# TaceoLabs/co-snarks

Measured on NVIDIA H100. Metric: co-Groth16 proofs/sec (BN254, 2^20 constraints); MSM Mscalar/s, higher is better.
Workload: dtype u32x8 (256-bit Montgomery, integer)

## Files before the change

co_snarks_b200/csrc/cs_api.cu:

```cuda
#include <stdarg.h>
#include "cs_lib.cuh"

namespace cs {

std::string& last_error() {
  static thread_local std::string e;
  return e;
}
int fail(int code, const char* fmt, ...) {
  char buf[1024];
  va_list ap;
  va_start(ap, fmt);
  vsnprintf(buf, sizeof(buf), fmt, ap);
  va_end(ap);
  last_error() = buf;
  return code;
}
#if !defined(CS_EMU)
__attribute__((constructor)) static void cs_more_hw_queues() { setenv("CUDA_DEVICE_MAX_CONNECTIONS", "32", 0); }
#endif

std::atomic<uint64_t>& launch_counter() {
  static std::atomic<uint64_t> c{0};
  return c;
// ... 155 lines not shown
int bases_upload_t(cs_ctx* ctx, const uint64_t* h_points, size_t n, int window_bits, cs_bases* b) {
  typedef typename GroupOf<Cfg, G>::F F;
  unsigned c = window_bits ? (unsigned)window_bits : msm_auto_window(n, Cfg::FR_BITS);
  if (c < 2 || c > MSM_MAX_WINDOW)
    return fail(CS_ERR_ARG, "cs_bases_upload: window_bits %d out of range [2,%u] (0 = automatic)", window_bits, MSM_MAX_WINDOW);
  b->sh = msm_shape(Cfg::FR_BITS, c);
  b->n = n;
  size_t total = (size_t)b->sh.W * n;
  if (total >= (1ull << 31)) return fail(CS_ERR_LIMIT, "cs_bases_upload: W*n = %zu exceeds 2^31", total);
  CS_TRY(b->table.reserve(total * sizeof(Affine<F>)));
  CS_CUDA(cudaMemcpyAsync(b->table.p, h_points, n * sizeof(Affine<F>), cudaMemcpyHostToDevice, ctx->stream));
  CS_TRY(b->infmask.reserve(((n + 31) / 32) * 4));
  CS_LAUNCH(k_msm_infmask<F>, ceil_div((n + 31) / 32, 128), 128, 0, ctx->stream, b->table.as<Affine<F>>(), (uint32_t)n,
            b->infmask.as<uint32_t>());
  CS_LAUNCH(k_msm_precompute<F>, ceil_div(n, 128), 128, 0, ctx->stream, b->table.as<Affine<F>>(), (uint32_t)n,
            b->sh.c, b->sh.W);
  if (G == 0 && std::is_same<Cfg, Bn254Cfg>::value) {
    static int f52_env = -1;
    if (f52_env < 0) { const char* e = getenv("CS_MSM_F52"); f52_env = e ? atoi(e) : 0; }
    if (f52_env) {
      const size_t ncoords = total * 2;
      CS_LAUNCH(k_msm_table_to_m260<Bn254Fq52 COMMA Bn254Fq>, ceil_div(ncoords, 128), 128, 0, ctx->stream,
                b->table.as<uint32_t>(), ncoords);
      b->m260 = true;
    }
  }
  CS_CUDA(cudaGetLastError());
  CS_CUDA(cudaStreamSynchronize(ctx->stream));
  return 0;
}

template <class Cfg, int G>
int msm_enqueue_t(cs_ctx* ctx, int slot, cudaStream_t st, const cs_bases* b, size_t offset,
                  const uint32_t* d_scalars, unsigned sstride, size_t n, int mont, int sort_slot, bool view) {
  typedef typename GroupOf<Cfg, G>::F F;
  return msm_enqueue<F, typename Cfg::FrP>(ctx->msm_ws[slot], b->table.as<Affine<F>>(), b->infmask.as<uint32_t>(), (uint32_t)b->n, b->sh,
                                           (uint32_t)offset, d_scalars, sstride, (uint32_t)n, mont, st,
                                           sort_slot >= 0 ? &ctx->msm_ws[sort_slot] : nullptr, view, b->m260, ctx->acc[slot]);
}

template <class Cfg, int G>
void msm_finish_t(cs_ctx* ctx, int slot, uint64_t* out_affine, int* out_inf) {
  typedef typename GroupOf<Cfg, G>::HF HF;
  const host::HXyzz<HF>* r = reinterpret_cast<const host::HXyzz<HF>*>(ctx->msm_ws[slot].h_result);
  host::HAffine<HF> a = host::haffine(*r);
  memcpy(out_affine, &a, sizeof(a));
  if (out_inf) *out_inf = a.is_inf() ? 1 : 0;
}

int msm_enqueue_dyn(cs_ctx* ctx, int slot, cudaStream_t st, const cs_bases* b, size_t offset,
                    const uint32_t* d_scalars, unsigned sstride, size_t n, int mont, int sort_slot, bool view) {
  CS_DISPATCH_CURVE(b->curve, {
    if (b->group == CS_G1) return msm_enqueue_t<Cfg, 0>(ctx, slot, st, b, offset, d_scalars, sstride, n, mont, sort_slot, view);
    return msm_enqueue_t<Cfg, 1>(ctx, slot, st, b, offset, d_scalars, sstride, n, mont, sort_slot, view);
  });
  return 0;
}
int msm_sort_shared_dyn(cs_ctx* ctx, int slot, cudaStream_t st, const cs_bases* b, const uint32_t* d_scalars,
                        unsigned sstride, size_t n, int mont) {
  CS_DISPATCH_CURVE(b->curve, {
    return msm_sort<typename Cfg::FrP>(ctx->msm_ws[slot], nullptr, (uint32_t)n, b->sh, 0, d_scalars, sstride, (uint32_t)n,
                                       mont, st);
  });
  return 0;
}

int msm_finish_dyn(cs_ctx* ctx, int slot, const cs_bases* b, uint64_t* out_affine, int* out_inf) {
  CS_DISPATCH_CURVE(b->curve, {
    if (b->group == CS_G1) msm_finish_t<Cfg, 0>(ctx, slot, out_affine, out_inf);
    else msm_finish_t<Cfg, 1>(ctx, slot, out_affine, out_inf);
  });
  return 0;
}

}

extern "C" {

int cs_bases_upload(cs_ctx* ctx, cs_curve curve, cs_group group, const uint64_t* h_points_mont, size_t n,
                    int window_bits, cs_bases** out) {
  if (!ctx || !h_points_mont || !out) return fail(CS_ERR_ARG, "cs_bases_upload: NULL argument");
  if (n == 0) return fail(CS_ERR_ARG, "cs_bases_upload: empty base set");
  if (group != CS_G1 && group != CS_G2) return fail(CS_ERR_ARG, "cs_bases_upload: bad group %d", (int)group);
  CS_CUDA(cudaSetDevice(ctx->device));
  std::unique_ptr<cs_bases> b(new cs_bases());
  b->curve = curve;
  b->group = group;
// ... 823 lines not shown
```

co_snarks_b200/csrc/cs_groth16.cu:

```cuda
#include <functional>
#include "cs_lib.cuh"
#include "cs_net.h"

using namespace cs;

struct cs_groth16_pk {
  int curve = 0;
  size_t nc = 0, ni = 0, nw = 0, n = 0;
  unsigned log_n = 0;
  DevBuf a_rowptr, a_col, a_coeff, b_rowptr, b_col, b_coeff;
  cs_bases *a_query = nullptr, *b_g1 = nullptr, *b_g2 = nullptr, *l_query = nullptr, *h_query = nullptr;
  std::vector<uint64_t> alpha_g1, beta_g1, beta_g2, delta_g1, delta_g2;
  std::vector<uint64_t> a_head, b1_head, b2_head;
  cs_domain* dom = nullptr;
  DevBuf coset_tab;
  DevBuf d_pub, d_wit, d_a, d_b, d_c, d_m1, d_m2;
  DevBuf c_rowptr, c_col, c_coeff;
  bool have_c = false;
  int wit_src[4] = {0, 1, 2, 3};
  cs_domain* dom_ark = nullptr;
  DevBuf coset_tab_ark, ginv_pows, vinv_over_n;
};

namespace {
// ... 209 lines not shown
      inf[j][i] = (words[k >> 5] >> (k & 31)) & 1;
      any = any || inf[j][i];
    }
    pk->wit_src[j] = j;
    if (q[j]->n == nw && off[j] == 0 && !any) {
      pk->wit_src[j] = -1;
      continue;
    }
    for (int k = 0; k < j; k++)
      if (pk->wit_src[k] == k && q[k]->n == q[j]->n && off[k] == off[j] && inf[k] == inf[j]) {
        pk->wit_src[j] = k;
        break;
      }
  }
  return 0;
}

int upload_inputs(cs_ctx* ctx, cs_groth16_pk* pk, int kind, const uint64_t* h_pub, const uint64_t* h_wit,
                  const uint64_t* h_m1, const uint64_t* h_m2) {
  const unsigned batch = kind == CS_REP3 ? 2 : 1;
  CS_TRY(upload(ctx, pk->d_pub, h_pub, pk->ni * 32));
  if (h_wit) CS_TRY(upload(ctx, pk->d_wit, h_wit, pk->nw * batch * 32));
  if (kind == CS_REP3 && h_m1) CS_TRY(upload(ctx, pk->d_m1, h_m1, pk->n * 32));
  if (kind == CS_REP3 && h_m2) CS_TRY(upload(ctx, pk->d_m2, h_m2, pk->n * 32));
  return 0;
}

template <class Cfg>
int local_phase(cs_ctx* ctx, cs_groth16_pk* pk, int kind, int party, const uint64_t* h_pub, const uint64_t* h_wit,
                const uint64_t* d_wit_in, const uint64_t* h_m1, const uint64_t* h_m2, const uint64_t* r_hs, const uint64_t* s_hs,
                uint64_t* out_a, uint64_t* out_b1, uint64_t* out_b2, uint64_t* out_l, uint64_t* out_h,
                unsigned parts = CS_PART_ALL, const cs_rep3_prf* prf = nullptr, const uint64_t* rs_mont = nullptr,
                uint64_t* out_rs_delta = nullptr, const std::function<void()>* overlap = nullptr,
                const std::function<int(const uint64_t*, const uint64_t*)>* mid = nullptr) {
  typedef HostGroup<Cfg, 0> H1;
  typedef HostGroup<Cfg, 1> H2;
  const unsigned batch = kind == CS_REP3 ? 2 : 1;
  const bool add_public = (kind == CS_PLAIN) || party == 0;
  const bool have_aux = pk->nw > 0;
  const bool do_a = parts & CS_PART_A, do_b1 = parts & CS_PART_B1, do_b2 = parts & CS_PART_B2,
             do_l = parts & CS_PART_L, do_h = parts & CS_PART_H;
  CS_CUDA(cudaSetDevice(ctx->device));
  CS_TRY(upload_inputs(ctx, pk, kind, h_pub, h_wit, do_h ? h_m1 : nullptr, do_h ? h_m2 : nullptr));
  CS_TRY(ctx_fork(ctx, 5));
  cudaStream_t wm = ctx->wm;
  CS_CUDA(cudaStreamWaitEvent(wm, ctx->ev_fork, 0));
  const uint32_t* wit = d_wit_in ? reinterpret_cast<const uint32_t*>(d_wit_in) : pk->d_wit.as<uint32_t>();
  if (do_h) {
    bool have_m1 = h_m1 != nullptr, have_m2 = h_m2 != nullptr;
    if (prf && kind == CS_REP3) {
      typedef typename Cfg::FrP FrP;
      const size_t n = pk->n;
      CS_TRY(pk->d_m1.reserve(n * 32));
      CS_TRY(pk->d_m2.reserve(n * 32));
      CS_TRY(ctx->prf_keys.reserve(64));
      CS_CUDA(cudaMemcpyAsync(ctx->prf_keys.p, prf->seed1, 32, cudaMemcpyHostToDevice, wm));
      CS_CUDA(cudaMemcpyAsync((char*)ctx->prf_keys.p + 32, prf->seed2, 32, cudaMemcpyHostToDevice, wm));
      CS_LAUNCH(k_rep3_masks<FrP>, ceil_div(n, 128), 128, 0, wm, ctx->prf_keys.as<uint32_t>(), prf->word_pos1,
                prf->word_pos2, prf->rounds, n, pk->d_m1.as<uint32_t>());
      CS_LAUNCH(k_rep3_masks<FrP>, ceil_div(n, 128), 128, 0, wm, ctx->prf_keys.as<uint32_t>(),
                prf->word_pos1 + 8 * n, prf->word_pos2 + 8 * n, prf->rounds, n, pk->d_m2.as<uint32_t>());
      have_m1 = have_m2 = true;
    }
    CS_TRY((witness_map_device<Cfg>(ctx, pk, kind, party, wit, have_m1, have_m2, wm)));
    {
      CS_SPAN("msm h_query");
      CS_TRY(msm_enqueue_dyn(ctx, 4, wm, pk->h_query, 0, pk->d_c.as<uint32_t>(), 1, pk->n, 1));
    }
  }
  if (have_aux) {
    CS_SPAN("compute A, B/G1, B/G2 in create proof with assignment + msm l_query");
    const unsigned part[4] = {CS_PART_A, CS_PART_B1, CS_PART_B2, CS_PART_L};
    const cs_bases* q[4] = {pk->a_query, pk->b_g1, pk->b_g2, pk->l_query};
    const size_t off[4] = {pk->ni, pk->ni, pk->ni, 0};
    if (do_a || do_b1 || do_b2 || do_l)
      CS_TRY(msm_sort_shared_dyn(ctx, CS_WIT_SORT, ctx->side[4], pk->a_query, wit, batch, pk->nw, 1));
    for (int j = 0; j < 4; j++) {
      if (!(parts & part[j])) continue;
      int src = pk->wit_src[j];
      if (src >= 0 && !(parts & part[src])) src = j;
      const int sort_slot = src < 0 || src == j ? CS_WIT_SORT : src;
      CS_TRY(msm_enqueue_dyn(ctx, j, ctx->side[j], q[j], off[j], wit, batch, pk->nw, 1, sort_slot, src == j));
    }
  }
  CS_TRY(ctx_join(ctx, 5));
  CS_CUDA(cudaEventRecord(ctx->ev_wm, wm));
  CS_CUDA(cudaStreamWaitEvent(ctx->stream, ctx->ev_wm, 0));

  const size_t g1l = 2 * H1::HF::N, g2l = 4 * H1::HF::N;
  typename H1::X a_acc = H1::X::inf(), b1_acc = H1::X::inf();
  typename H2::X b2_acc = H2::X::inf();
  if (do_a) {
    a_acc = H1::mul(H1::load(pk->delta_g1.data()), r_hs);
    if (add_public) {
      a_acc = host::hadd(a_acc, H1::load(pk->a_head.data()));
      a_acc = host::hadd(a_acc, H1::load(pk->alpha_g1.data()));
      for (size_t k = 1; k < pk->ni; k++)
        a_acc = host::hadd(a_acc, H1::mul(H1::load(pk->a_head.data() + k * g1l), h_pub + k * 4));
    }
  }
  if (do_b1) {
    b1_acc = H1::mul(H1::load(pk->delta_g1.data()), s_hs);
    if (add_public) {
      b1_acc = host::hadd(b1_acc, H1::load(pk->b1_head.data()));
      b1_acc = host::hadd(b1_acc, H1::load(pk->beta_g1.data()));
      for (size_t k = 1; k < pk->ni; k++)
        b1_acc = host::hadd(b1_acc, H1::mul(H1::load(pk->b1_head.data() + k * g1l), h_pub + k * 4));
    }
  }
  if (do_b2) {
    b2_acc = H2::mul(H2::load(pk->delta_g2.data()), s_hs);
    if (add_public) {
      b2_acc = host::hadd(b2_acc, H2::load(pk->b2_head.data()));
      b2_acc = host::hadd(b2_acc, H2::load(pk->beta_g2.data()));
      for (size_t k = 1; k < pk->ni; k++)
        b2_acc = host::hadd(b2_acc, H2::mul(H2::load(pk->b2_head.data() + k * g2l), h_pub + k * 4));
    }
  }
  CS_SPAN("r*s without networking");
  if (rs_mont && out_rs_delta)
    H1::store(out_rs_delta, H1::mul(H1::load(pk->delta_g1.data()), rs_mont));
  if (overlap) (*overlap)();
  uint64_t tmp[24];
  int inf = 0;
  bool ab_done = false;
  if (mid && have_aux && do_a && do_b1) {
    CS_CUDA(cudaEventSynchronize(ctx->ev_side[0]));
    CS_CUDA(cudaEventSynchronize(ctx->ev_side[1]));
    CS_TRY(msm_finish_dyn(ctx, 0, pk->a_query, tmp, &inf)); a_acc = host::hadd(a_acc, H1::load(tmp));
    CS_TRY(msm_finish_dyn(ctx, 1, pk->b_g1, tmp, &inf)); b1_acc = host::hadd(b1_acc, H1::load(tmp));
    H1::store(out_a, a_acc);
    H1::store(out_b1, b1_acc);
    CS_TRY((*mid)(out_a, out_b1));
    ab_done = true;
  }
  CS_CUDA(cudaStreamSynchronize(ctx->stream));
  memset(out_l, 0, g1l * 8);
  memset(out_h, 0, g1l * 8);
  if (have_aux) {
    if (do_a && !ab_done) { CS_TRY(msm_finish_dyn(ctx, 0, pk->a_query, tmp, &inf)); a_acc = host::hadd(a_acc, H1::load(tmp)); }
    if (do_b1 && !ab_done) { CS_TRY(msm_finish_dyn(ctx, 1, pk->b_g1, tmp, &inf)); b1_acc = host::hadd(b1_acc, H1::load(tmp)); }
    if (do_b2) { CS_TRY(msm_finish_dyn(ctx, 2, pk->b_g2, tmp, &inf)); b2_acc = host::hadd(b2_acc, H2::load(tmp)); }
    if (do_l) CS_TRY(msm_finish_dyn(ctx, 3, pk->l_query, out_l, &inf));
  }
  if (do_h) CS_TRY(msm_finish_dyn(ctx, 4, pk->h_query, out_h, &inf));
  if (!ab_done) {
    H1::store(out_a, a_acc);
    H1::store(out_b1, b1_acc);
  }
  H2::store(out_b2, b2_acc);
  if (mid && !ab_done) CS_TRY((*mid)(out_a, out_b1));
  return 0;
}

template <class Cfg>
int prove_plain_t(cs_ctx* ctx, cs_groth16_pk* pk, const uint64_t* h_pub, const uint64_t* h_wit,
                  const uint64_t* d_wit, const uint64_t* r, const uint64_t* s, uint64_t* out_a, uint64_t* out_b,
                  uint64_t* out_c) {
  typedef HostGroup<Cfg, 0> H1;
  typedef host::HFp<typename Cfg::FrP> HR;
  uint64_t a[12], b1[12], l[12], h[12], rsd[12];
  HR rr, ss;
  memcpy(rr.l, r, sizeof(rr.l));
  memcpy(ss.l, s, sizeof(ss.l));
  HR rs = rr * ss;
  typename H1::X c = H1::X::inf();
  std::function<int(const uint64_t*, const uint64_t*)> mid = [&](const uint64_t* pa, const uint64_t* pb1) -> int {
    c = host::hadd(H1::mul(H1::load(pa), s), H1::mul(H1::load(pb1), r));
    return 0;
  };
  CS_TRY((local_phase<Cfg>(ctx, pk, CS_PLAIN, 0, h_pub, h_wit, d_wit, nullptr, nullptr, r, s, a, b1, out_b, l, h,
                           CS_PART_ALL, nullptr, rs.l, rsd, nullptr, &mid)));
  c = host::hadd(c, host::hneg(H1::load(rsd)));
  c = host::hadd(c, H1::load(l));
  c = host::hadd(c, H1::load(h));
  memcpy(out_a, a, 2 * H1::HF::N * 8);
  H1::store(out_c, c);
  return 0;
}


template <class Cfg>
int rep3_prove_t(cs_ctx* ctx, cs_groth16_pk* pk, cs_net* net0, cs_net* net1, cs_net* pair, int role, int party,
                 cs_rep3_state* state0, const uint64_t* h_pub, const uint64_t* h_wit, const uint64_t* d_wit,
                 uint64_t* out_a, uint64_t* out_b, uint64_t* out_c, uint64_t* out_rs) {
  typedef HostGroup<Cfg, 0> H1;
  typedef HostGroup<Cfg, 1> H2;
  typedef host::HFp<typename Cfg::FrP> HR;
  typedef typename Cfg::FrP FrP;
  constexpr size_t G1L = 2 * H1::HF::N, G2L = 4 * H1::HF::N;
  const size_t n = pk->n;
  cs_rep3_state* st1p = nullptr;
  CS_TRY(cs_rep3_state_fork(state0, &st1p));
  std::unique_ptr<cs_rep3_state> state1(st1p);
  cs_rep3_prf prf;
  CS_TRY(cs_rep3_state_prf(state0, &prf));
  CS_TRY(cs_rep3_state_advance(state0, 16 * (uint64_t)n));
  uint64_t r_sh[2 * HR::N], s_sh[2 * HR::N];
  CS_TRY(cs_rep3_state_rand(state0, (cs_curve)pk->curve, r_sh));
  CS_TRY(cs_rep3_state_rand(state0, (cs_curve)pk->curve, s_sh));
  if (out_rs) { memcpy(out_rs, r_sh, sizeof(r_sh)); memcpy(out_rs + 2 * HR::N, s_sh, sizeof(s_sh)); }
  HR ra, rb, sa, sb;
  memcpy(ra.l, r_sh, sizeof(ra.l)); memcpy(rb.l, r_sh + HR::N, sizeof(rb.l));
  memcpy(sa.l, s_sh, sizeof(sa.l)); memcpy(sb.l, s_sh + HR::N, sizeof(sb.l));
  HR m1 = state0->rng1.template fr_be_mod_order<FrP>(), m2 = state0->rng2.template fr_be_mod_order<FrP>();
// ... 10 lines not shown
    memcpy(msg + G2L, h, G1L * 8);
    return cs_net_send(pair, 0, msg, sizeof(msg));
  }
  typename H1::X ec_mask = H1::X::inf();
  std::function<void()> overlap = [&]() {
    typename H1::X g = H1::load(pk->alpha_g1.data());
    HR a1, a2;
    memcpy(a1.l, k1, sizeof(a1.l)); memcpy(a2.l, k2, sizeof(a2.l));
    HR d = a1 - a2;
    HR dc = d.from_mont();
    ec_mask = host::hmul(g, dc.l, HR::N);
  };
  uint64_t g_a[G1L], g1_b[G1L], g2_b[G2L], l_acc[G1L], h_acc[G1L], rsd[G1L];
  const unsigned parts = role == 1 ? (CS_PART_A | CS_PART_B1 | CS_PART_L) : CS_PART_ALL;
  Rep3Net n0(net0), n1(net1);
  typename H1::X A_open = H1::X::inf(), g_c = H1::X::inf();
  std::function<int(const uint64_t*, const uint64_t*)> mid = [&](const uint64_t* pa, const uint64_t* pb1) -> int {
    CS_SPAN("network round after calc coeff");
    CS_TRY(n0.send_next(pa, G1L * 8));
    CS_TRY(n0.send_prev(pa, G1L * 8));
    CS_TRY(n1.send_next(pb1, G1L * 8));
    typename H1::X B1 = H1::load(pb1);
    typename H1::X t = H1::mul(B1, r_sh + HR::N);
    uint64_t ga_prev[G1L], ga_next[G1L], g1b_prev[G1L];
    CS_TRY(n0.recv_prev(ga_prev, G1L * 8));
    CS_TRY(n0.recv_next(ga_next, G1L * 8));
    CS_TRY(n1.recv_prev(g1b_prev, G1L * 8));
    A_open = host::hadd(host::hadd(H1::load(pa), H1::load(ga_prev)), H1::load(ga_next));
    typename H1::X r_g1_b = host::hadd(host::hadd(H1::mul(host::hadd(B1, H1::load(g1b_prev)), r_sh), t), ec_mask);
    g_c = host::hadd(H1::mul(A_open, s_sh), r_g1_b);
    return 0;
  };
  CS_TRY((local_phase<Cfg>(ctx, pk, CS_REP3, party, h_pub, h_wit, d_wit, nullptr, nullptr, r_sh, s_sh, g_a, g1_b, g2_b,
                           l_acc, h_acc, parts, role == 1 ? nullptr : &prf, rs.l, rsd, &overlap, &mid)));
  if (role == 1) {
    uint64_t msg[G2L + G1L];
    CS_TRY(cs_net_recv(pair, 1, msg, sizeof(msg)));
    memcpy(g2_b, msg, G2L * 8);
    memcpy(h_acc, msg + G2L, G1L * 8);
  }
  CS_SPAN("finish - open two points and some adds");
  g_c = host::hadd(g_c, host::hneg(H1::load(rsd)));
  g_c = host::hadd(g_c, H1::load(l_acc));
  g_c = host::hadd(g_c, H1::load(h_acc));
  uint64_t gc[G1L];
  H1::store(gc, g_c);
  CS_TRY(n0.send_next(gc, G1L * 8));
  CS_TRY(n0.send_prev(gc, G1L * 8));
  CS_TRY(n1.send_next(g2_b, G2L * 8));
  CS_TRY(n1.send_prev(g2_b, G2L * 8));
  uint64_t gc_prev[G1L], gc_next[G1L], b2_prev[G2L], b2_next[G2L];
  CS_TRY(n0.recv_prev(gc_prev, G1L * 8));
  CS_TRY(n0.recv_next(gc_next, G1L * 8));
  CS_TRY(n1.recv_prev(b2_prev, G2L * 8));
  CS_TRY(n1.recv_next(b2_next, G2L * 8));
  H1::store(out_a, A_open);
  H1::store(out_c, host::hadd(host::hadd(g_c, H1::load(gc_prev)), H1::load(gc_next)));
  H2::store(out_b, host::hadd(host::hadd(H2::load(g2_b), H2::load(b2_prev)), H2::load(b2_next)));
  return 0;
}

template <class Cfg>
int shamir_prove_t(cs_ctx* ctx, cs_groth16_pk* pk, cs_net* net0, cs_net* net1, int n_parties, int threshold,
                   const uint64_t* h_pub, const uint64_t* h_wit, const uint64_t* d_wit, uint64_t* out_a, uint64_t* out_b,
                   uint64_t* out_c, uint64_t* out_rs) {
  typedef HostGroup<Cfg, 0> H1;
  typedef host::HFp<typename Cfg::FrP> HR;
  constexpr size_t G1L = 2 * H1::HF::N, G2L = 4 * H1::HF::N;
  cs_shamir_state* s0 = nullptr;
  CS_TRY(cs_shamir_state_create(net0, (cs_curve)pk->curve, n_parties, threshold, 3, &s0));
  struct Guard { cs_shamir_state* a = nullptr; cs_shamir_state* b = nullptr; ~Guard() { cs_shamir_state_free(a); cs_shamir_state_free(b); } } guard;
  guard.a = s0;
  cs_shamir_state* s1 = nullptr;
  CS_TRY(cs_shamir_state_fork(s0, 1, &s1));
  guard.b = s1;
  uint64_t r[HR::N], sv[HR::N];
  CS_TRY(cs_shamir_state_rand(s0, net0, r));
  CS_TRY(cs_shamir_state_rand(s0, net0, sv));
  if (out_rs) { memcpy(out_rs, r, sizeof(r)); memcpy(out_rs + HR::N, sv, sizeof(sv)); }
  HR rr, ss;
  memcpy(rr.l, r, sizeof(r));
  memcpy(ss.l, sv, sizeof(sv));
  HR rs = rr * ss;
  uint64_t g_a[G1L], g1_b[G1L], g2_b[G2L], l_acc[G1L], h_acc[G1L], rsd[G1L];
  CS_TRY((local_phase<Cfg>(ctx, pk, CS_PLAIN, 0, h_pub, h_wit, d_wit, nullptr, nullptr, r, sv, g_a, g1_b, g2_b, l_acc, h_acc,
                           CS_PART_ALL, nullptr, rs.l, rsd)));
  uint64_t a_open[G1L], g1_b_red[G1L];
  CS_TRY(cs_shamir_open_half_point(s0, net0, CS_G1, g_a, a_open));
  CS_TRY(cs_shamir_degree_reduce_point(s1, net1, CS_G1, pk->alpha_g1.data(), g1_b, g1_b_red));
  typename H1::X r_g1_b = H1::mul(H1::load(g1_b_red), r);
  typename H1::X g_c = H1::mul(H1::load(a_open), sv);
  g_c = host::hadd(g_c, r_g1_b);
  g_c = host::hadd(g_c, host::hneg(H1::load(rsd)));
  g_c = host::hadd(g_c, H1::load(l_acc));
  g_c = host::hadd(g_c, H1::load(h_acc));
  uint64_t gc[G1L];
  H1::store(gc, g_c);
  CS_TRY(cs_shamir_open_half_point(s0, net0, CS_G1, gc, out_c));
  CS_TRY(cs_shamir_open_half_point(s1, net1, CS_G2, g2_b, out_b));
  memcpy(out_a, a_open, sizeof(a_open));
  return 0;
}

int rep3_prove_dispatch(cs_ctx* ctx, cs_groth16_pk* pk, cs_net* net0, cs_net* net1, cs_net* pair, int role, int party,
                        cs_rep3_state* state, const uint64_t* h_pub, const uint64_t* h_wit, const uint64_t* d_wit,
                        uint64_t* out_a, uint64_t* out_b, uint64_t* out_c, uint64_t* out_rs) {
  if (!ctx || !pk || !state || !h_pub) return fail(CS_ERR_ARG, "cs_groth16_rep3_prove: NULL argument");
  if (pk->nw && !h_wit == !d_wit) return fail(CS_ERR_ARG, "cs_groth16_rep3_prove: pass the witness shares either on the host or on the device");
  if (role != 2) {
    if (!net0 || !net1 || !out_a || !out_b || !out_c) return fail(CS_ERR_ARG, "cs_groth16_rep3_prove: NULL argument");
    if (net0->n != 3 || net1->n != 3 || net0->id != net1->id) return fail(CS_ERR_ARG, "cs_groth16_rep3_prove: net0/net1 must be 3-party meshes of the same party");
    if (net0->id != state->id) return fail(CS_ERR_ARG, "cs_groth16_rep3_prove: state belongs to party %d, net to party %d", state->id, net0->id);
  }
  if (role != 0 && (!pair || pair->n != 2 || pair->id != role - 1)) return fail(CS_ERR_ARG, "cs_groth16_rep3_prove: pair must be the 2-party link (id %d)", role - 1);
  if (party < 0 || party > 2) return fail(CS_ERR_ARG, "cs_groth16_rep3_prove: party must be 0..2");
  switch (pk->curve) {
    case CS_BN254:
      return rep3_prove_t<Bn254Cfg>(ctx, pk, net0, net1, pair, role, party, state, h_pub, h_wit, d_wit, out_a, out_b, out_c, out_rs);
#if defined(CS_ENABLE_BLS12_381)
// ... 314 lines not shown
```

co_snarks_b200/csrc/cs_lib.cuh:

```cuda
#pragma once
#include <atomic>
#include <map>
#include <memory>
#include "cs_common.cuh"
#include "cs_params.cuh"
#include "cs_curve.cuh"
#include "cs_msm.cuh"
#include "cs_msm52.cuh"
#include "cs_ntt.cuh"
#include "cs_ntt8.cuh"
#include "cs_vec.cuh"
#include "cs_prf.cuh"
#include "cs_host_field.h"
#include "../../include/cosnarks_gpu.h"

namespace cs {

struct Bn254Cfg {
  typedef Bn254Fq FqP;
  typedef Bn254Fr FrP;
  static constexpr unsigned FR_BITS = 254;
  static constexpr unsigned TWO_ADICITY = 28;
};
struct Bls381Cfg {
// ... 52 lines not shown
  unsigned log_n = 0;
  cs::DevBuf tw_fwd, tw_inv;
  cs::DevBuf inv_n;
  std::vector<uint64_t> group_gen;
};

#if defined(CS_ENABLE_BLS12_381)
#define CS_CASE_BLS(...)   \
  case CS_BLS12_381: {     \
    typedef Bls381Cfg Cfg; \
    __VA_ARGS__;           \
  } break;
#else
#define CS_CASE_BLS(...)
#endif

#define CS_DISPATCH_CURVE(curve, ...)                                        \
  switch ((int)(curve)) {                                                    \
    case CS_BN254: {                                                         \
      typedef Bn254Cfg Cfg;                                                  \
      __VA_ARGS__;                                                           \
    } break;                                                                 \
      CS_CASE_BLS(__VA_ARGS__)                                               \
    default:                                                                 \
      return cs::fail(CS_ERR_ARG, "unsupported curve id %d", (int)(curve));      \
  }


namespace cs {
std::atomic<uint64_t>& launch_counter();
int ctx_fork(cs_ctx* ctx, int nside);
int ctx_join(cs_ctx* ctx, int nside);
int msm_enqueue_dyn(cs_ctx* ctx, int slot, cudaStream_t st, const cs_bases* b, size_t offset,
                    const uint32_t* d_scalars, unsigned sstride, size_t n, int mont, int sort_slot = -1, bool view = false);
int msm_sort_shared_dyn(cs_ctx* ctx, int slot, cudaStream_t st, const cs_bases* b, const uint32_t* d_scalars,
                        unsigned sstride, size_t n, int mont);
int msm_finish_dyn(cs_ctx* ctx, int slot, const cs_bases* b, uint64_t* out_affine, int* out_inf);
int ntt_run(cs_ctx* ctx, const cs_domain* d, uint32_t* d_data, unsigned batch, bool inverse_in_to_out,
            const uint32_t* d_post, cudaStream_t st);
}
```

co_snarks_b200/csrc/cs_msm.cuh:

```cuda
#pragma once
#include <stdlib.h>
#include "cs_common.cuh"
#include "cs_curve.cuh"

namespace cs {

constexpr unsigned MSM_SLICE_MAX = 64;
constexpr unsigned MSM_ORDER_BLOCK = 256;
constexpr unsigned MSM_RED_SEG = 4;
constexpr unsigned MSM_SIGN = 0x80000000u;

template <class FrP>
CS_GLOBAL void k_msm_digits(const uint32_t* __restrict__ scalars, uint32_t sstride, uint32_t n, int mont,
                            uint32_t c, uint32_t W, const uint32_t* __restrict__ infmask, uint32_t offset,
                            uint32_t* __restrict__ dig, uint32_t* __restrict__ count) {
  uint32_t i = blockIdx.x * blockDim.x + threadIdx.x;
  if (i >= n) return;
  if (infmask && ((infmask[(offset + i) >> 5] >> ((offset + i) & 31)) & 1)) {
    for (uint32_t w = 0; w < W; w++) dig[(size_t)w * n + i] = 0;
    return;
  }
  Fp<FrP> s;
  const uint4* src = reinterpret_cast<const uint4*>(scalars) + (size_t)i * sstride * (FrP::N / 4);
  CS_UNROLL
// ... 351 lines not shown
  }
  Affine<F> p = table[e & ~MSM_SIGN];
  for (uint32_t k = beg; k < end; k++) {
    uint32_t e_cur = e;
    Affine<F> p_cur = p;
    if (k + 1 < end) {
      e = sorted[k + 1];
      p = table[e & ~MSM_SIGN];
    }
    madd(acc, p_cur, (e_cur & MSM_SIGN) != 0);
  }
  part0[s] = acc;
}

template <class F>
CS_GLOBAL void __launch_bounds__(128) k_msm_accum1(const Xyzz<F>* __restrict__ part0,
                                                   const uint32_t* __restrict__ sstart0,
                                                   const uint32_t* __restrict__ sstart1, uint32_t nb1, uint32_t S,
                                                   Xyzz<F>* __restrict__ part1) {
  uint32_t s = blockIdx.x * blockDim.x + threadIdx.x;
  if (s >= sstart1[nb1]) return;
  uint32_t b = find_bucket(sstart1, nb1, s);
  uint32_t j = s - sstart1[b];
  uint32_t beg = sstart0[b] + j * S;
  uint32_t end = sstart0[b + 1];
  if (end > beg + S) end = beg + S;
  Xyzz<F> acc = part0[beg];
  for (uint32_t k = beg + 1; k < end; k++) padd(acc, part0[k]);
  part1[s] = acc;
}

template <class F>
CS_GLOBAL void __launch_bounds__(128) k_msm_accum2(const Xyzz<F>* __restrict__ part1,
                                                   const uint32_t* __restrict__ sstart1, uint32_t nb1,
                                                   Xyzz<F>* __restrict__ bucket) {
  uint32_t b = blockIdx.x * blockDim.x + threadIdx.x;
  if (b >= nb1) return;
  uint32_t beg = sstart1[b], end = sstart1[b + 1];
  Xyzz<F> acc = Xyzz<F>::inf();
  if (beg < end) {
    acc = part1[beg];
    for (uint32_t k = beg + 1; k < end; k++) padd(acc, part1[k]);
  }
  bucket[b] = acc;
}

template <class F>
CS_GLOBAL void __launch_bounds__(128) k_msm_reduce_seg(const Xyzz<F>* __restrict__ bucket, uint32_t B,
                                                       uint32_t L, Xyzz<F>* __restrict__ red) {
  uint32_t t = blockIdx.x * blockDim.x + threadIdx.x;
  uint32_t lo = t * L;
  if (lo >= B) return;
  uint32_t hi = lo + L < B ? lo + L : B;
  Xyzz<F> acc = Xyzz<F>::inf(), tot = Xyzz<F>::inf();
  for (uint32_t b = hi; b > lo; b--) {
    padd(acc, bucket[b]);
    padd(tot, acc);
  }
  if (lo != 0 && !acc.is_inf()) {
    Xyzz<F> m = Xyzz<F>::inf();
    int top = 31 - __clz(lo);
    for (int bit = top; bit >= 0; bit--) {
      m = dbl_xyzz(m);
      if ((lo >> bit) & 1) padd(m, acc);
    }
    padd(tot, m);
  }
  red[t] = tot;
}

template <class F>
CS_GLOBAL void k_msm_final_sum(const Xyzz<F>* __restrict__ red, uint32_t cnt,
                                                      Xyzz<F>* __restrict__ out) {
  CS_DYN_SMEM(Xyzz<F>, sm);
  const uint32_t T = blockDim.x, t = threadIdx.x;
  Xyzz<F> acc = Xyzz<F>::inf();
// ... 81 lines not shown
  Xyzz<F> acc = Xyzz<F>::inf();
  for (int bit = FrP::N * 32 - 1; bit >= 0; bit--) {
    acc = dbl_xyzz(acc);
    if ((lim[bit >> 5] >> (bit & 31)) & 1) madd(acc, b, false);
  }
  out[i] = to_affine(acc);
}

struct MsmShape {
  uint32_t c, W, B;
};

static inline MsmShape msm_shape(uint32_t scalar_bits, uint32_t c) {
  MsmShape s;
  s.c = c;
  s.W = (scalar_bits + 1 + c - 1) / c;
  s.B = 1u << (c - 1);
  return s;
}

static inline uint32_t msm_auto_window(size_t n, uint32_t scalar_bits) {
  int lg = 0;
  while ((1ull << (lg + 1)) <= n) lg++;
  int c = lg >= 15 ? 16 : lg - 4;
  if (c < 4) c = 4;
  while (c < 16) {
    const uint32_t W = (scalar_bits + 1 + c - 1) / c;
    const uint32_t top = scalar_bits + 1 - (W - 1) * c;
    if (2 * top >= (uint32_t)c) break;
    c++;
  }
  return (uint32_t)c;
}
static inline uint32_t msm_slice(const MsmShape& sh) {
  const char* e = getenv("CS_MSM_SLICE");
  if (e && atoi(e) == 64) return 64u;
  if (e && atoi(e) == 32) return 32u;
  return sh.c >= 18 ? 64u : 32u;
}

constexpr int MSM_NSTAGE = 5;
struct MsmWorkspace {
  DevBuf dig, sorted, meta, part0, part1, part2, bucket, red, scal, result, order;
  void* h_result = nullptr;
  size_t h_result_cap = 0;
  bool profile = false;
  cudaEvent_t ev[MSM_NSTAGE + 1] = {};
  cudaEvent_t sorted_ev = nullptr;
  bool sorted_ev_made = false, sorted_once = false;
  cudaEvent_t acc_in = nullptr, acc_out = nullptr;
  int mark(int i, cudaStream_t st) {
    if (!profile) return 0;
    if (!ev[i]) CS_CUDA(cudaEventCreateWithFlags(&ev[i], 0));
    CS_CUDA(cudaEventRecord(ev[i], st));
    return 0;
  }
  void release() {
    for (int i = 0; i <= MSM_NSTAGE; i++) {
      if (ev[i]) cudaEventDestroy(ev[i]);
      ev[i] = nullptr;
    }
    if (sorted_ev_made) cudaEventDestroy(sorted_ev);
    if (acc_in) cudaEventDestroy(acc_in);
    if (acc_out) cudaEventDestroy(acc_out);
    acc_in = acc_out = nullptr;
    sorted_ev = nullptr;
    sorted_ev_made = sorted_once = false;
    dig.release(); sorted.release(); meta.release(); part0.release(); part1.release(); part2.release();
    bucket.release(); red.release(); scal.release(); result.release(); order.release();
    if (h_result) cudaFreeHost(h_result);
    h_result = nullptr;
    h_result_cap = 0;
  }
};

template <class F>
int msm_accum0_f52(const Affine<F>* table, const uint32_t* sorted, const uint32_t* count, const uint32_t* start,
                   const uint32_t* sstart0, uint32_t nb1, uint32_t S, const uint32_t* order, const uint32_t* order_b,
                   Xyzz<F>* part0, uint32_t max_s0, cudaStream_t st);

struct MsmSizes {
  uint32_t nb1, S, ob;
  size_t nent, max_s0, max_s1, max_s2;
  MsmSizes(const MsmShape& sh, uint32_t n) {
    nb1 = sh.B + 1;
    nent = (size_t)sh.W * n;
    S = msm_slice(sh);
    max_s0 = nent / S + nb1;
    max_s1 = max_s0 / S + nb1;
    max_s2 = max_s1 / S + nb1;
    ob = ceil_div(max_s0, MSM_ORDER_BLOCK);
  }
  size_t meta_words() const { return 2 * (size_t)nb1 + 4 * ((size_t)nb1 + 1) + 4 * MSM_SCAN_MAX_BLOCKS; }
  size_t order_words() const {
    return 4 * max_s0 + (size_t)ob * (MSM_SLICE_MAX + 1) + 2 * (MSM_SLICE_MAX + 1) + (size_t)(MSM_SLICE_MAX + 1) * MSM_OFF_CHUNKS;
  }
};
struct MsmSortBufs {
  uint32_t *count, *cursor, *start, *sstart0, *sstart1, *sstart2, *aux;
  uint32_t *slice_len, *slice_bkt, *order, *order_b, *block_hist, *len_base, *chunk_sum;
  MsmSortBufs(const MsmWorkspace& w, const MsmSizes& z) {
    count = w.meta.as<uint32_t>();
    cursor = count + z.nb1;
    start = cursor + z.nb1;
    sstart0 = start + z.nb1 + 1;
    sstart1 = sstart0 + z.nb1 + 1;
    sstart2 = sstart1 + z.nb1 + 1;
    aux = sstart2 + z.nb1 + 1;
    slice_len = w.order.as<uint32_t>();
    slice_bkt = slice_len + z.max_s0;
    order = slice_bkt + z.max_s0;
    order_b = order + z.max_s0;
    block_hist = order_b + z.max_s0;
    len_base = block_hist + (size_t)z.ob * (MSM_SLICE_MAX + 1);
    chunk_sum = len_base + 2 * (MSM_SLICE_MAX + 1);
  }
};

static inline int msm_check_limits(const MsmShape& sh, uint32_t n, uint32_t nbases) {
  const size_t nent = (size_t)sh.W * n;
// ... 45 lines not shown
  CS_TRY(ws.mark(1, st));
  CS_TRY(msm_scan(q, z, sh.B, st));
  CS_LAUNCH(k_msm_scatter, dim3(ceil_div(n, 256), sh.W), 256, 0, st, ws.dig.as<uint32_t>(), n, nbases, offset, q.start,
            q.cursor, ws.sorted.as<uint32_t>());
  return msm_slice_order(ws, q, z, st);
}

static inline int msm_view(MsmWorkspace& ws, const MsmWorkspace& src, const uint32_t* infmask, uint32_t nbases,
                           MsmShape sh, uint32_t offset, uint32_t n, cudaStream_t st) {
  const MsmSizes z(sh, n);
  const uint32_t nblk = ceil_div(z.nent, MSM_VIEW_T);
  CS_TRY(ws.dig.reserve(((size_t)nblk * MSM_VIEW_WORDS + 2 * (size_t)nblk + 1) * 4));
  CS_TRY(ws.sorted.reserve(z.nent * 4));
  CS_TRY(ws.meta.reserve(z.meta_words() * 4));
  CS_TRY(ws.order.reserve(z.order_words() * 4));
  const MsmSortBufs q(ws, z), s(src, z);
  uint32_t* keep = ws.dig.as<uint32_t>();
  uint32_t* blk_cnt = keep + (size_t)nblk * MSM_VIEW_WORDS;
  uint32_t* blk_off = blk_cnt + nblk;
  const uint32_t* src_sorted = src.sorted.as<uint32_t>();
  CS_LAUNCH_SYNC(k_msm_view_flags, nblk, MSM_VIEW_T, 0, st, src_sorted, s.start, z.nb1, n, infmask, offset, keep, blk_cnt);
  CS_LAUNCH_SYNC(k_msm_view_scan, 1, MSM_SCAN_T, 0, st, blk_cnt, nblk, blk_off);
  CS_LAUNCH(k_msm_view_counts, ceil_div(z.nb1, 256), 256, 0, st, s.start, z.nb1, keep, blk_off, q.count);
  CS_LAUNCH(k_msm_view_scatter, nblk, MSM_VIEW_T, 0, st, src_sorted, n, nbases, offset, keep, blk_off,
            ws.sorted.as<uint32_t>());
  CS_TRY(msm_scan(q, z, sh.B, st));
  return msm_slice_order(ws, q, z, st);
}

template <class F, class FrP>
int msm_enqueue(MsmWorkspace& ws, const Affine<F>* table, const uint32_t* infmask, uint32_t nbases, MsmShape sh,
                uint32_t offset,
                const uint32_t* d_scalars, uint32_t sstride, uint32_t n, int mont, cudaStream_t st,
                MsmWorkspace* sort_from = nullptr, bool view = false, bool table_m260 = false, cudaStream_t st_acc = nullptr) {
  CS_TRY(msm_check_limits(sh, n, nbases));
  const MsmSizes z(sh, n);
  const uint32_t nb1 = z.nb1, S = z.S;
  const size_t max_s0 = z.max_s0, max_s1 = z.max_s1, max_s2 = z.max_s2;
  CS_TRY(ws.part0.reserve(max_s0 * sizeof(Xyzz<F>)));
  CS_TRY(ws.part1.reserve(max_s1 * sizeof(Xyzz<F>)));
  CS_TRY(ws.part2.reserve(max_s2 * sizeof(Xyzz<F>)));
  CS_TRY(ws.bucket.reserve((size_t)nb1 * sizeof(Xyzz<F>)));
  const uint32_t L = sh.B < MSM_RED_SEG ? sh.B : MSM_RED_SEG;
  const uint32_t nseg = (sh.B + L - 1) / L;
  const uint32_t fs_threads = sizeof(Xyzz<F>) > 128 ? 128 : 256;
  const uint32_t fs_blocks = nseg > 4 * fs_threads ? (nseg + fs_threads - 1) / fs_threads : 1;
  CS_TRY(ws.red.reserve(((size_t)nseg + fs_blocks) * sizeof(Xyzz<F>)));
  CS_TRY(ws.result.reserve(sizeof(Xyzz<F>)));
  if (ws.h_result_cap < sizeof(Xyzz<F>)) {
    if (ws.h_result) cudaFreeHost(ws.h_result);
    CS_CUDA(cudaMallocHost(&ws.h_result, sizeof(Xyzz<F>)));
    ws.h_result_cap = sizeof(Xyzz<F>);
  }
  if (sort_from) {
    if (!sort_from->sorted_once) return fail(-1, "msm: the workspace to share a sort with has not been enqueued");
    CS_TRY(ws.mark(0, st));
    CS_CUDA(cudaStreamWaitEvent(st, sort_from->sorted_ev, 0));
    CS_TRY(ws.mark(1, st));
    if (view) CS_TRY(msm_view(ws, *sort_from, infmask, nbases, sh, offset, n, st));
  } else {
    CS_TRY(msm_sort<FrP>(ws, infmask, nbases, sh, offset, d_scalars, sstride, n, mont, st));
  }
  MsmWorkspace& so = sort_from && !view ? *sort_from : ws;
  const MsmSortBufs q(so, z);
  const uint32_t *count = q.count, *start = q.start, *sstart0 = q.sstart0, *sstart1 = q.sstart1, *sstart2 = q.sstart2;
  const uint32_t *order = q.order, *order_b = q.order_b;
  CS_TRY(ws.mark(2, st));
// ... 8 lines not shown
    st = st_acc;
  }
  {
    static int minb_env = -1;
    if (minb_env < 0) { const char* e = getenv("CS_ACCUM0_MINB"); minb_env = e ? atoi(e) : 0; }
    const int minb = minb_env ? minb_env : (sizeof(Affine<F>) > 64 ? 2 : 4);
    if (table_m260) {
      CS_TRY((msm_accum0_f52<F>(table, so.sorted.as<uint32_t>(), count, start, sstart0, nb1, S, order, order_b,
                                ws.part0.as<Xyzz<F>>(), (uint32_t)max_s0, st)));
    } else {
#define CS_ACC0(M)                                                                                              \
  CS_LAUNCH(k_msm_accum0<F COMMA M>, ceil_div(max_s0, 128), 128, 0, st, table, so.sorted.as<uint32_t>(), count, \
            start, sstart0, nb1, S, order, order_b, ws.part0.as<Xyzz<F>>())
    switch (minb) {
      case 2: CS_ACC0(2); break;
      case 3: CS_ACC0(3); break;
      case 5: CS_ACC0(5); break;
      case 6: CS_ACC0(6); break;
      default: CS_ACC0(4); break;
    }
#undef CS_ACC0
    }
  }
  if (st_acc) {
    CS_CUDA(cudaEventRecord(ws.acc_out, st_acc));
    st = st_main;
    CS_CUDA(cudaStreamWaitEvent(st, ws.acc_out, 0));
  }
  CS_TRY(ws.mark(3, st));
  CS_LAUNCH(k_msm_accum1<F>, ceil_div(max_s1, 128), 128, 0, st, ws.part0.as<Xyzz<F>>(), sstart0, sstart1,
            nb1, S, ws.part1.as<Xyzz<F>>());
  CS_LAUNCH(k_msm_accum1<F>, ceil_div(max_s2, 128), 128, 0, st, ws.part1.as<Xyzz<F>>(), sstart1, sstart2,
            nb1, S, ws.part2.as<Xyzz<F>>());
  CS_LAUNCH(k_msm_accum2<F>, ceil_div(nb1, 128), 128, 0, st, ws.part2.as<Xyzz<F>>(), sstart2, nb1,
            ws.bucket.as<Xyzz<F>>());
  CS_TRY(ws.mark(4, st));
  CS_LAUNCH(k_msm_reduce_seg<F>, ceil_div(nseg, 128), 128, 0, st, ws.bucket.as<Xyzz<F>>(), sh.B, L,
            ws.red.as<Xyzz<F>>());
  if (fs_blocks > 1) {
    Xyzz<F>* stage = ws.red.as<Xyzz<F>>() + nseg;
    CS_LAUNCH_SYNC(k_msm_final_sum<F>, fs_blocks, fs_threads, fs_threads * sizeof(Xyzz<F>), st, ws.red.as<Xyzz<F>>(), nseg,
                   stage);
    CS_LAUNCH_SYNC(k_msm_final_sum<F>, 1, fs_threads, fs_threads * sizeof(Xyzz<F>), st, stage, fs_blocks,
                   ws.result.as<Xyzz<F>>());
  } else {
    CS_LAUNCH_SYNC(k_msm_final_sum<F>, 1, fs_threads, fs_threads * sizeof(Xyzz<F>), st, ws.red.as<Xyzz<F>>(), nseg,
                   ws.result.as<Xyzz<F>>());
  }
  CS_TRY(ws.mark(5, st));
  CS_CUDA(cudaMemcpyAsync(ws.h_result, ws.result.p, sizeof(Xyzz<F>), cudaMemcpyDeviceToHost, st));
  CS_CUDA(cudaGetLastError());
  return 0;
}

}
```

Measured before the change: 49.69.

## Fold H-query MSM partial buckets into L-query MSM to share reduction tail

Result: faster. 50.73, median of 6 (+2.1%).

```diff
diff --git a/co_snarks_b200/csrc/cs_api.cu b/co_snarks_b200/csrc/cs_api.cu
--- a/co_snarks_b200/csrc/cs_api.cu
+++ b/co_snarks_b200/csrc/cs_api.cu
@@ -211,11 +211,13 @@
 
 template <class Cfg, int G>
 int msm_enqueue_t(cs_ctx* ctx, int slot, cudaStream_t st, const cs_bases* b, size_t offset,
-                  const uint32_t* d_scalars, unsigned sstride, size_t n, int mont, int sort_slot, bool view) {
+                  const uint32_t* d_scalars, unsigned sstride, size_t n, int mont, int sort_slot, bool view,
+                  bool defer_tail, int fold_slot) {
   typedef typename GroupOf<Cfg, G>::F F;
   return msm_enqueue<F, typename Cfg::FrP>(ctx->msm_ws[slot], b->table.as<Affine<F>>(), b->infmask.as<uint32_t>(), (uint32_t)b->n, b->sh,
                                            (uint32_t)offset, d_scalars, sstride, (uint32_t)n, mont, st,
-                                           sort_slot >= 0 ? &ctx->msm_ws[sort_slot] : nullptr, view, b->m260, ctx->acc[slot]);
+                                           sort_slot >= 0 ? &ctx->msm_ws[sort_slot] : nullptr, view, b->m260, ctx->acc[slot],
+                                           defer_tail, fold_slot >= 0 ? &ctx->msm_ws[fold_slot] : nullptr);
 }
 
 template <class Cfg, int G>
@@ -228,10 +230,12 @@
 }
 
 int msm_enqueue_dyn(cs_ctx* ctx, int slot, cudaStream_t st, const cs_bases* b, size_t offset,
-                    const uint32_t* d_scalars, unsigned sstride, size_t n, int mont, int sort_slot, bool view) {
+                    const uint32_t* d_scalars, unsigned sstride, size_t n, int mont, int sort_slot, bool view,
+                    bool defer_tail, int fold_slot) {
   CS_DISPATCH_CURVE(b->curve, {
-    if (b->group == CS_G1) return msm_enqueue_t<Cfg, 0>(ctx, slot, st, b, offset, d_scalars, sstride, n, mont, sort_slot, view);
-    return msm_enqueue_t<Cfg, 1>(ctx, slot, st, b, offset, d_scalars, sstride, n, mont, sort_slot, view);
+    if (b->group == CS_G1)
+      return msm_enqueue_t<Cfg, 0>(ctx, slot, st, b, offset, d_scalars, sstride, n, mont, sort_slot, view, defer_tail, fold_slot);
+    return msm_enqueue_t<Cfg, 1>(ctx, slot, st, b, offset, d_scalars, sstride, n, mont, sort_slot, view, defer_tail, fold_slot);
   });
   return 0;
 }
diff --git a/co_snarks_b200/csrc/cs_groth16.cu b/co_snarks_b200/csrc/cs_groth16.cu
--- a/co_snarks_b200/csrc/cs_groth16.cu
+++ b/co_snarks_b200/csrc/cs_groth16.cu
@@ -265,7 +265,7 @@
                 uint64_t* out_a, uint64_t* out_b1, uint64_t* out_b2, uint64_t* out_l, uint64_t* out_h,
                 unsigned parts = CS_PART_ALL, const cs_rep3_prf* prf = nullptr, const uint64_t* rs_mont = nullptr,
                 uint64_t* out_rs_delta = nullptr, const std::function<void()>* overlap = nullptr,
-                const std::function<int(const uint64_t*, const uint64_t*)>* mid = nullptr) {
+                const std::function<int(const uint64_t*, const uint64_t*)>* mid = nullptr, bool sum_lh = false) {
   typedef HostGroup<Cfg, 0> H1;
   typedef HostGroup<Cfg, 1> H2;
   const unsigned batch = kind == CS_REP3 ? 2 : 1;
@@ -273,6 +273,8 @@
   const bool have_aux = pk->nw > 0;
   const bool do_a = parts & CS_PART_A, do_b1 = parts & CS_PART_B1, do_b2 = parts & CS_PART_B2,
              do_l = parts & CS_PART_L, do_h = parts & CS_PART_H;
+  const bool merge_lh = sum_lh && have_aux && do_l && do_h && pk->l_query->sh.c == pk->h_query->sh.c &&
+                        pk->l_query->sh.W == pk->h_query->sh.W;
   CS_CUDA(cudaSetDevice(ctx->device));
   CS_TRY(upload_inputs(ctx, pk, kind, h_pub, h_wit, do_h ? h_m1 : nullptr, do_h ? h_m2 : nullptr));
   CS_TRY(ctx_fork(ctx, 5));
@@ -298,7 +300,7 @@
     CS_TRY((witness_map_device<Cfg>(ctx, pk, kind, party, wit, have_m1, have_m2, wm)));
     {
       CS_SPAN("msm h_query");
-      CS_TRY(msm_enqueue_dyn(ctx, 4, wm, pk->h_query, 0, pk->d_c.as<uint32_t>(), 1, pk->n, 1));
+      CS_TRY(msm_enqueue_dyn(ctx, 4, wm, pk->h_query, 0, pk->d_c.as<uint32_t>(), 1, pk->n, 1, -1, false, merge_lh));
     }
   }
   if (have_aux) {
@@ -313,7 +315,8 @@
       int src = pk->wit_src[j];
       if (src >= 0 && !(parts & part[src])) src = j;
       const int sort_slot = src < 0 || src == j ? CS_WIT_SORT : src;
-      CS_TRY(msm_enqueue_dyn(ctx, j, ctx->side[j], q[j], off[j], wit, batch, pk->nw, 1, sort_slot, src == j));
+      CS_TRY(msm_enqueue_dyn(ctx, j, ctx->side[j], q[j], off[j], wit, batch, pk->nw, 1, sort_slot, src == j, false,
+                             j == 3 && merge_lh ? 4 : -1));
     }
   }
   CS_TRY(ctx_join(ctx, 5));
@@ -376,7 +379,7 @@
     if (do_b2) { CS_TRY(msm_finish_dyn(ctx, 2, pk->b_g2, tmp, &inf)); b2_acc = host::hadd(b2_acc, H2::load(tmp)); }
     if (do_l) CS_TRY(msm_finish_dyn(ctx, 3, pk->l_query, out_l, &inf));
   }
-  if (do_h) CS_TRY(msm_finish_dyn(ctx, 4, pk->h_query, out_h, &inf));
+  if (do_h && !merge_lh) CS_TRY(msm_finish_dyn(ctx, 4, pk->h_query, out_h, &inf));
   if (!ab_done) {
     H1::store(out_a, a_acc);
     H1::store(out_b1, b1_acc);
@@ -403,7 +406,7 @@
     return 0;
   };
   CS_TRY((local_phase<Cfg>(ctx, pk, CS_PLAIN, 0, h_pub, h_wit, d_wit, nullptr, nullptr, r, s, a, b1, out_b, l, h,
-                           CS_PART_ALL, nullptr, rs.l, rsd, nullptr, &mid)));
+                           CS_PART_ALL, nullptr, rs.l, rsd, nullptr, &mid, true)));
   c = host::hadd(c, host::hneg(H1::load(rsd)));
   c = host::hadd(c, H1::load(l));
   c = host::hadd(c, H1::load(h));
@@ -480,7 +483,7 @@
     return 0;
   };
   CS_TRY((local_phase<Cfg>(ctx, pk, CS_REP3, party, h_pub, h_wit, d_wit, nullptr, nullptr, r_sh, s_sh, g_a, g1_b, g2_b,
-                           l_acc, h_acc, parts, role == 1 ? nullptr : &prf, rs.l, rsd, &overlap, &mid)));
+                           l_acc, h_acc, parts, role == 1 ? nullptr : &prf, rs.l, rsd, &overlap, &mid, true)));
   if (role == 1) {
     uint64_t msg[G2L + G1L];
     CS_TRY(cs_net_recv(pair, 1, msg, sizeof(msg)));
@@ -532,7 +535,7 @@
   HR rs = rr * ss;
   uint64_t g_a[G1L], g1_b[G1L], g2_b[G2L], l_acc[G1L], h_acc[G1L], rsd[G1L];
   CS_TRY((local_phase<Cfg>(ctx, pk, CS_PLAIN, 0, h_pub, h_wit, d_wit, nullptr, nullptr, r, sv, g_a, g1_b, g2_b, l_acc, h_acc,
-                           CS_PART_ALL, nullptr, rs.l, rsd)));
+                           CS_PART_ALL, nullptr, rs.l, rsd, nullptr, nullptr, true)));
   uint64_t a_open[G1L], g1_b_red[G1L];
   CS_TRY(cs_shamir_open_half_point(s0, net0, CS_G1, g_a, a_open));
   CS_TRY(cs_shamir_degree_reduce_point(s1, net1, CS_G1, pk->alpha_g1.data(), g1_b, g1_b_red));
diff --git a/co_snarks_b200/csrc/cs_lib.cuh b/co_snarks_b200/csrc/cs_lib.cuh
--- a/co_snarks_b200/csrc/cs_lib.cuh
+++ b/co_snarks_b200/csrc/cs_lib.cuh
@@ -108,7 +108,8 @@
 int ctx_fork(cs_ctx* ctx, int nside);
 int ctx_join(cs_ctx* ctx, int nside);
 int msm_enqueue_dyn(cs_ctx* ctx, int slot, cudaStream_t st, const cs_bases* b, size_t offset,
-                    const uint32_t* d_scalars, unsigned sstride, size_t n, int mont, int sort_slot = -1, bool view = false);
+                    const uint32_t* d_scalars, unsigned sstride, size_t n, int mont, int sort_slot = -1, bool view = false,
+                    bool defer_tail = false, int fold_slot = -1);
 int msm_sort_shared_dyn(cs_ctx* ctx, int slot, cudaStream_t st, const cs_bases* b, const uint32_t* d_scalars,
                         unsigned sstride, size_t n, int mont);
 int msm_finish_dyn(cs_ctx* ctx, int slot, const cs_bases* b, uint64_t* out_affine, int* out_inf);
diff --git a/co_snarks_b200/csrc/cs_msm.cuh b/co_snarks_b200/csrc/cs_msm.cuh
--- a/co_snarks_b200/csrc/cs_msm.cuh
+++ b/co_snarks_b200/csrc/cs_msm.cuh
@@ -407,7 +407,9 @@
 
 template <class F>
 CS_GLOBAL void __launch_bounds__(128) k_msm_accum2(const Xyzz<F>* __restrict__ part1,
-                                                   const uint32_t* __restrict__ sstart1, uint32_t nb1,
+                                                   const uint32_t* __restrict__ sstart1,
+                                                   const Xyzz<F>* __restrict__ part_b,
+                                                   const uint32_t* __restrict__ sstart_b, uint32_t nb1,
                                                    Xyzz<F>* __restrict__ bucket) {
   uint32_t b = blockIdx.x * blockDim.x + threadIdx.x;
   if (b >= nb1) return;
@@ -417,6 +419,8 @@
     acc = part1[beg];
     for (uint32_t k = beg + 1; k < end; k++) padd(acc, part1[k]);
   }
+  if (part_b)
+    for (uint32_t k = sstart_b[b]; k < sstart_b[b + 1]; k++) padd(acc, part_b[k]);
   bucket[b] = acc;
 }
 
@@ -564,11 +568,11 @@
   }
   return (uint32_t)c;
 }
-static inline uint32_t msm_slice(const MsmShape& sh) {
+static inline uint32_t msm_slice(const MsmShape& sh, size_t nent) {
   const char* e = getenv("CS_MSM_SLICE");
   if (e && atoi(e) == 64) return 64u;
   if (e && atoi(e) == 32) return 32u;
-  return sh.c >= 18 ? 64u : 32u;
+  return sh.c >= 18 || (sh.c >= 16 && nent >= 255 * (size_t)sh.B) ? 64u : 32u;
 }
 
 constexpr int MSM_NSTAGE = 5;
@@ -581,6 +585,10 @@
   cudaEvent_t sorted_ev = nullptr;
   bool sorted_ev_made = false, sorted_once = false;
   cudaEvent_t acc_in = nullptr, acc_out = nullptr;
+  cudaEvent_t part_ev = nullptr;
+  bool part_ev_made = false;
+  const uint32_t* part_sstart2 = nullptr;
+  uint32_t part_nb1 = 0;
   int mark(int i, cudaStream_t st) {
     if (!profile) return 0;
     if (!ev[i]) CS_CUDA(cudaEventCreateWithFlags(&ev[i], 0));
@@ -595,7 +603,11 @@
     if (sorted_ev_made) cudaEventDestroy(sorted_ev);
     if (acc_in) cudaEventDestroy(acc_in);
     if (acc_out) cudaEventDestroy(acc_out);
-    acc_in = acc_out = nullptr;
+    if (part_ev_made) cudaEventDestroy(part_ev);
+    acc_in = acc_out = part_ev = nullptr;
+    part_ev_made = false;
+    part_sstart2 = nullptr;
+    part_nb1 = 0;
     sorted_ev = nullptr;
     sorted_ev_made = sorted_once = false;
     dig.release(); sorted.release(); meta.release(); part0.release(); part1.release(); part2.release();
@@ -617,7 +629,7 @@
   MsmSizes(const MsmShape& sh, uint32_t n) {
     nb1 = sh.B + 1;
     nent = (size_t)sh.W * n;
-    S = msm_slice(sh);
+    S = msm_slice(sh, nent);
     max_s0 = nent / S + nb1;
     max_s1 = max_s0 / S + nb1;
     max_s2 = max_s1 / S + nb1;
@@ -729,7 +741,8 @@
 int msm_enqueue(MsmWorkspace& ws, const Affine<F>* table, const uint32_t* infmask, uint32_t nbases, MsmShape sh,
                 uint32_t offset,
                 const uint32_t* d_scalars, uint32_t sstride, uint32_t n, int mont, cudaStream_t st,
-                MsmWorkspace* sort_from = nullptr, bool view = false, bool table_m260 = false, cudaStream_t st_acc = nullptr) {
+                MsmWorkspace* sort_from = nullptr, bool view = false, bool table_m260 = false, cudaStream_t st_acc = nullptr,
+                bool defer_tail = false, MsmWorkspace* fold_in = nullptr) {
   CS_TRY(msm_check_limits(sh, n, nbases));
   const MsmSizes z(sh, n);
   const uint32_t nb1 = z.nb1, S = z.S;
@@ -804,7 +817,29 @@
             nb1, S, ws.part1.as<Xyzz<F>>());
   CS_LAUNCH(k_msm_accum1<F>, ceil_div(max_s2, 128), 128, 0, st, ws.part1.as<Xyzz<F>>(), sstart1, sstart2,
             nb1, S, ws.part2.as<Xyzz<F>>());
-  CS_LAUNCH(k_msm_accum2<F>, ceil_div(nb1, 128), 128, 0, st, ws.part2.as<Xyzz<F>>(), sstart2, nb1,
+  if (defer_tail) {
+    if (!ws.part_ev_made) {
+      CS_CUDA(cudaEventCreateWithFlags(&ws.part_ev, cudaEventDisableTiming));
+      ws.part_ev_made = true;
+    }
+    CS_CUDA(cudaEventRecord(ws.part_ev, st));
+    ws.part_sstart2 = sstart2;
+    ws.part_nb1 = nb1;
+    CS_TRY(ws.mark(4, st));
+    CS_TRY(ws.mark(5, st));
+    CS_CUDA(cudaGetLastError());
+    return 0;
+  }
+  const Xyzz<F>* part_b = nullptr;
+  const uint32_t* sstart_b = nullptr;
+  if (fold_in) {
+    if (!fold_in->part_ev_made || fold_in->part_nb1 != nb1)
+      return fail(-1, "msm: the MSM to fold in has not been enqueued with this MSM's window");
+    CS_CUDA(cudaStreamWaitEvent(st, fold_in->part_ev, 0));
+    part_b = fold_in->part2.as<Xyzz<F>>();
+    sstart_b = fold_in->part_sstart2;
+  }
+  CS_LAUNCH(k_msm_accum2<F>, ceil_div(nb1, 128), 128, 0, st, ws.part2.as<Xyzz<F>>(), sstart2, part_b, sstart_b, nb1,
             ws.bucket.as<Xyzz<F>>());
   CS_TRY(ws.mark(4, st));
   CS_LAUNCH(k_msm_reduce_seg<F>, ceil_div(nseg, 128), 128, 0, st, ws.bucket.as<Xyzz<F>>(), sh.B, L,
```
